# Ouranosinc/xclim

Measured on AMD Instinct MI355X. Metric: grid-cells x timesteps / s (tx90p = percentile_doy + threshold_count + missing mask), higher is better.
Workload: dtype f32; 1 GPU; tx90p (percentile_doy window 5 per 90 + threshold_count > + MissingAny) on 365x1440x720 fp32 per GPU, noleap, freq YS, time-major, resident in HBM

## Files before the change

xclim_amd/csrc/common.h:

```cpp
#pragma once
#include <hip/hip_runtime.h>
#include <stdint.h>
#include <stdio.h>
#include <string.h>

#include "../../include/xclim_hip.h"

struct xh_ctx {
  int device;
  hipStream_t stream;
  hipEvent_t ev0, ev1;
  hipStream_t stream2;
  hipEvent_t ev_ready[2], ev_done[2];
  hipStream_t copy_in, copy_out;
  hipEvent_t ev_lane;
  void* scratch;
  size_t scratch_bytes;
  char* scratch_host;
  size_t scratch_head;
  void* retired[16];
  char* retired_host[16];
  int nretired;
  void* big;
  size_t big_bytes;
// ... 12 lines not shown
    if (_e != hipSuccess) {                                                                 \
      xh_set_error("%s failed: %s (%s:%d)", #expr, hipGetErrorString(_e), __FILE__, __LINE__); \
      (void)hipGetLastError();   \
      return XH_ERR_HIP;                                                                    \
    }                                                                                       \
  } while (0)

#define XH_REQUIRE(cond, code, ...) \
  do {                              \
    if (!(cond)) {                  \
      xh_set_error(__VA_ARGS__);    \
      return (code);                \
    }                               \
  } while (0)

#define XH_LAUNCH_CHECK()                                                                      \
  do {                                                                                         \
    hipError_t _e = hipGetLastError();                                                         \
    if (_e != hipSuccess) {                                                                    \
      xh_set_error("kernel launch failed: %s (%s:%d)", hipGetErrorString(_e), __FILE__, __LINE__); \
      return XH_ERR_HIP;                                                                       \
    }                                                                                          \
  } while (0)

int xh_nanmax_fix(xh_ctx* ctx, const float* x, int64_t T, int64_t C, int64_t st, int64_t sc, int nq, float* out);
int xh_correction_fix(xh_ctx* ctx, const float* ref, const float* hist, int64_t T, int64_t C, int64_t st, int64_t sc, int nq, int kind,
                      float* af, float* hist_q);
int xh_scratch_upload(xh_ctx* ctx, size_t* cursor, const void* host, size_t bytes, void** dptr);
int xh_big_scratch(xh_ctx* ctx, size_t bytes, void** dptr);
int xh_const_rows(xh_ctx* ctx, int64_t elems, const float** nan_row, const float** ninf_row, const float** pinf_row);
int xh_launch_tcount_doy(xh_ctx* ctx, const float* x, int64_t T, int64_t C, int64_t st, int op, const double* table,
                         int64_t tstride, const int32_t* tidx, const int64_t* d_seg, const int64_t* h_seg, int P, int ndoy,
                         int32_t* count_out, int32_t* valid_out);
int xh_qdm_columns(xh_ctx* ctx, const float* xcols, int64_t T, int64_t ncols, int64_t col_stride, const float* af, int64_t af_qs,
                   const double* d_q, int nq, int kind, int interp, int extrap, float* out, int64_t out_cs);
int xh_qdm_sorted_ws(int64_t T, int64_t ncols, size_t* bytes);
int xh_qdm_sorted(xh_ctx* ctx, const float* xcols, int64_t T, int64_t ncols, int64_t col_stride, const float* af, int64_t af_qs,
                  const double* d_q, int nq, int kind, int interp, int extrap, float* out, int64_t out_cs, void* ws);
int xh_qdm_regsort(xh_ctx* ctx, const float* sim, int64_t T, int64_t C, int64_t st, const float* af, int64_t af_qs,
                   const double* d_q, int nq, int kind, int extrap, float* scen, int64_t ost);
int xh_cut_classify(xh_ctx* ctx, const float* sim, int64_t T, int64_t C, int64_t st, const float* gcut, const float* gfac, int ntest,
                    int kind, float* scen, int64_t ost);
int xh_qdm_hist(xh_ctx* ctx, const float* sim, int64_t T, int64_t C, int64_t st, const float* af, int64_t af_qs, const double* d_q,
                int nq, int kind, int extrap, float* scen, int64_t ost);
int xh_tcount_plan(int64_t T, int64_t C, int64_t st, int op, int P, int ndoy, int64_t longest, size_t* lds, int* narrow);
int64_t xh_tcount_meta_slots(int64_t T);
int64_t xh_tcount_slot_of_row(int64_t t);
int xh_tcount_run(xh_ctx* ctx, const float* x, int64_t T, int64_t C, int64_t st, int op, const double* table, int64_t tstride,
                  const uint32_t* meta, int P, int ndoy, int narrow, size_t lds, int32_t* count_out, int32_t* valid_out);
int xh_select_columns(xh_ctx* ctx, const float* xcols, int64_t T, int64_t ncols, int64_t col_stride, const double* d_q,
                      int nq, float* out, int64_t out_cstride, int64_t out_qstride);
int xh_select_columns_lean(xh_ctx* ctx, const float* xcols, int64_t T, int64_t ncols, int64_t col_stride,
                           const double* d_q, int nq, float* out, int64_t out_cstride, int64_t out_qstride);
int xh_select_columns_radix(xh_ctx* ctx, const float* xcols, int64_t T, int64_t ncols, int64_t col_stride, const double* d_q,
                            int nq, float* out, int64_t out_cstride, int64_t out_qstride);
int xh_select_regsort(xh_ctx* ctx, const float* x, int64_t T, int64_t C, int64_t st, const double* d_q, int nq, float* out,
                      int64_t out_cstride, int64_t out_qstride);
int xh_select_hist(xh_ctx* ctx, const float* x, int64_t T, int64_t C, int64_t st, const double* d_q, int nq, float* out,
                   int64_t out_cstride, int64_t out_qstride);
int xh_select_time_major(xh_ctx* ctx, const float* x, int64_t T, int64_t C, int64_t st, const double* d_q, int nq,
                         float* out, int64_t out_cstride, int64_t out_qstride);

__host__ __device__ static inline int64_t cdiv64(int64_t a, int64_t b) { return (a + b - 1) / b; }

#define XH_BLOCK 256

// ... 212 lines not shown
```

xclim_amd/csrc/quantile.hip:

```cpp
#include <stdlib.h>

#include <type_traits>

#include "pdoy.h"

template <typename Getter>
__device__ __forceinline__ double xh_hf_quantile(int L, int n, double q, double alpha, double beta, Getter get) {
  if (L == 1) return (double)get(0);
  if (n < 2) {
    return n == 1 ? (double)get(0) : xh_nan64();
  }
  double nn = (double)n;
  double vi = nn * q + (alpha + q * (1.0 - alpha - beta)) - 1.0;
  if (vi >= nn - 1.0) return (double)get(n - 1);
  if (vi < 0.0) {
    const float v0 = get(0);
    return (v0 - v0 != 0.0f) ? (double)get(n - 1) : (double)v0;
  }
  double prev = floor(vi);
  int ip = (int)prev;
  double gamma = vi - prev;
  float left = get(ip), right = get(ip + 1);
  float diff = right - left;
  double r = (double)left + (double)diff * gamma;
// ... 67 lines not shown
        return xh_key2f(r);
      };
      for (int j = 0; j < nper; ++j) {
        double r = xh_hf_quantile(N, nvalid[v], qs[j], alpha, beta, get);
        out[((int64_t)j * ndoy + d) * C + c + v] = r;
      }
    }
  }
}

__device__ __forceinline__ void ce(uint32_t& a, uint32_t& b) {
  uint32_t lo = a < b ? a : b, hi = a < b ? b : a;
  a = lo;
  b = hi;
}

template <int W>
__device__ __forceinline__ void sort_small(uint32_t (&k)[W]) {
  if (W == 1) return;
  if (W == 2) { ce(k[0], k[1 % W]); return; }
  if (W == 3) { ce(k[0], k[1 % W]); ce(k[1 % W], k[2 % W]); ce(k[0], k[1 % W]); return; }
  if (W == 5) {
    ce(k[0], k[1 % W]); ce(k[3 % W], k[4 % W]); ce(k[2 % W], k[4 % W]); ce(k[2 % W], k[3 % W]); ce(k[0], k[3 % W]);
    ce(k[0], k[2 % W]); ce(k[1 % W], k[4 % W]); ce(k[1 % W], k[3 % W]); ce(k[1 % W], k[2 % W]);
    return;
  }
#pragma unroll
  for (int r = 0; r < W; ++r) {
#pragma unroll
    for (int i = (r & 1); i + 1 < W; i += 2) ce(k[i], k[i + 1]);
  }
}

template <int W, int VEC, bool COUNT = false>
__global__ void __launch_bounds__(XH_BLOCK)
k_pdoy_slide(const float* __restrict__ x, int64_t T, int64_t C, int64_t st, int64_t t_first, int ndoy, int chunk,
             const QTab* __restrict__ qtab, int nper, double* __restrict__ out, int fast, int op = 0,
             const int32_t* __restrict__ doy_period = nullptr, int32_t* __restrict__ cnt_out = nullptr,
             int32_t* __restrict__ valid_out = nullptr) {
  __shared__ QTab s_tab[8 * (W + 1)];
  for (int i = threadIdx.x; i < nper * (W + 1); i += XH_BLOCK) s_tab[i] = qtab[i];
  __syncthreads();
  constexpr int NP = VEC == 4 ? 2 : 1;
  constexpr int GW = VEC == 4 ? 2 : 1;
  const int lane = threadIdx.x & 63;
  const int64_t wbase = ((int64_t)blockIdx.x * XH_BLOCK + (threadIdx.x & ~63)) * VEC;
  if (wbase >= C) return;
  int64_t cg[NP];
  bool okg[NP];
#pragma unroll
  for (int g = 0; g < NP; ++g) {
    cg[g] = wbase + (VEC == 4 ? 2 * lane + 128 * g : lane);
    okg[g] = cg[g] < C;
  }
  auto cell = [&](int v) -> int64_t { return cg[v / GW] + v % GW; };
  constexpr int half = W / 2;
  int d0 = blockIdx.y * chunk, d1 = d0 + chunk;
  if (d1 > ndoy) d1 = ndoy;
  uint32_t win[VEC][W];
  int n[VEC];
#pragma unroll
  for (int v = 0; v < VEC; ++v) {
    n[v] = 0;
#pragma unroll
    for (int k = 0; k < W; ++k) win[v][k] = 0xFFFFFFFFu;
  }
  auto fetch = [&](int64_t t) -> VecF<VEC> {
    const int64_t tc = t < 0 ? 0 : (t >= T ? T - 1 : t);
    const float* row = x + tc * st;
    VecF<VEC> r;
#pragma unroll
    for (int g = 0; g < NP; ++g) {
      const VecF<GW> h = xh_load<GW>(row + (okg[g] ? cg[g] : C - GW));
#pragma unroll
// ... 499 lines not shown
    hipLaunchKernelGGL((k_pdoy_reg<16, 1>), grid, dim3(XH_BLOCK), 0, ctx->stream, x, T, C, st, d_tbase, nyears, ndoy,
                       window, d_q, nper, alpha, beta, out);
  } else if (N <= 32) {
    dim3 grid((unsigned)cdiv64(C, XH_BLOCK), gy);
    hipLaunchKernelGGL((k_pdoy_reg<32, 1>), grid, dim3(XH_BLOCK), 0, ctx->stream, x, T, C, st, d_tbase, nyears, ndoy,
                       window, d_q, nper, alpha, beta, out);
  } else {
    return launch_pdoy_lds(ctx, x, T, C, st, d_tbase, nyears, ndoy, window, d_q, nper, alpha, beta, out, nullptr, T, nullptr,
                           0);
  }
  XH_LAUNCH_CHECK();
  return XH_OK;
}

static int slide_fast_mode(const QTab* tab, int nper, int W) {
  bool allmax = W > 1, allmin = W > 1;
  for (int j = 0; j < nper; ++j) {
    const QTab& e = tab[j * (W + 1) + W];
    allmax = allmax && e.lo == e.hi && e.lo == W - 1;
    allmin = allmin && e.lo == e.hi && e.lo == 0;
  }
  return allmax ? 1 : (allmin ? 2 : 0);
}

static int pdoy_impl(xh_ctx* ctx, const float* x, int64_t T, int64_t C, int64_t st, const int32_t* tbase, int nyears,
                     int ndoy, int window, const double* qh, int nper, double alpha, double beta, const int32_t* vmap,
                     int64_t Tv, double* out) {
  size_t cur = 0;
  void *d_tb = nullptr, *d_q = nullptr, *d_vmap = nullptr;
  const int N = nyears * window;
  bool contiguous = !vmap && nyears == 1 && nper <= 8 && (window == 3 || window == 5 || window == 7) && tbase[0] >= 0;
  for (int d = 1; contiguous && d < ndoy; ++d) contiguous = tbase[d] == tbase[0] + d;
  if (contiguous) {
    QTab tab[8 * 8];
    build_qtab(window, qh, nper, alpha, beta, tab);
    void* d_tab = nullptr;
    int rc = xh_scratch_upload(ctx, &cur, tab, sizeof(QTab) * (size_t)nper * (window + 1), &d_tab);
    if (rc) return rc;
    int chunk = 32;
    if (const char* e = xh_diag_env("XH_PDOY_SLIDE_CHUNK")) chunk = atoi(e) > 0 ? atoi(e) : chunk;
    const int vec = slide_vec(x, C, st, out);
    dim3 grid((unsigned)cdiv64(cdiv64(C, vec), XH_BLOCK), (unsigned)((ndoy + chunk - 1) / chunk));
#define XH_SLIDE(W, V)                                                                                              \
  hipLaunchKernelGGL((k_pdoy_slide<W, V>), grid, dim3(XH_BLOCK), 0, ctx->stream, x, T, C, st, (int64_t)tbase[0], ndoy, \
                     chunk, (const QTab*)d_tab, nper, out, slide_fast_mode(tab, nper, window))
    if (vec == 4) {
      if (window == 3) XH_SLIDE(3, 4); else if (window == 5) XH_SLIDE(5, 4); else XH_SLIDE(7, 4);
    } else {
      if (window == 3) XH_SLIDE(3, 1); else if (window == 5) XH_SLIDE(5, 1); else XH_SLIDE(7, 1);
    }
#undef XH_SLIDE
    XH_LAUNCH_CHECK();
    return XH_OK;
  }
  int rc = xh_scratch_upload(ctx, &cur, tbase, sizeof(int32_t) * (size_t)nyears * ndoy, &d_tb);
  if (rc) return rc;
  rc = xh_scratch_upload(ctx, &cur, qh, sizeof(double) * nper, &d_q);
  if (rc) return rc;
  if (vmap) {
    rc = xh_scratch_upload(ctx, &cur, vmap, sizeof(int32_t) * (size_t)Tv, &d_vmap);
    if (rc) return rc;
  }
  if (!vmap && N <= 32)
    return launch_pdoy(ctx, x, T, C, st, (const int32_t*)d_tb, nyears, ndoy, window, (const double*)d_q, nper, alpha, beta,
                       out);
  const bool mergeable = N > 32 && nyears <= 64 && (window == 3 || window == 5 || window == 7) && nper <= 16;
  if (!mergeable)
    return launch_pdoy_lds(ctx, x, T, C, st, (const int32_t*)d_tb, nyears, ndoy, window, (const double*)d_q, nper, alpha,
                           beta, out, (const int32_t*)d_vmap, Tv, nullptr, 0);
  uint8_t* regular = (uint8_t*)malloc((size_t)ndoy);
  int32_t* irregular = (int32_t*)malloc(sizeof(int32_t) * (size_t)ndoy);
  QTab* tab = (QTab*)malloc(sizeof(QTab) * (size_t)nper * (N + 1));
  if (!regular || !irregular || !tab) {
    free(regular); free(irregular); free(tab);
    xh_set_error("xh_percentile_doy: out of host memory");
    return XH_ERR_ARG;
  }
  const int nirr = pdoy_regular_flags(tbase, nyears, ndoy, window, T, vmap, Tv, regular, irregular);
// ... 76 lines not shown
                                         hipFuncAttributeMaxDynamicSharedMemorySize, (int)lds));                           \
      hipLaunchKernelGGL((k_pdoy_merge<W, NY, false>), grid, dim3(64), lds, ctx->stream, x, T, C, st, (const int32_t*)d_tb, \
                         nyears, ndoy, chunk, (const QTab*)d_tab, (const int32_t*)d_jrest, nrest, out,                      \
                         (const int32_t*)d_vmap, Tv, (const uint8_t*)d_reg, (const int32_t*)nullptr, 0, KT, KB, abl);       \
    }                                                                                                                      \
    if (nirr) {                                                                                                            \
      if (lds_a > 64 * 1024)                                                                                               \
        XH_CHECK_HIP(hipFuncSetAttribute((const void*)k_pdoy_merge<W, NY, true>,                                           \
                                         hipFuncAttributeMaxDynamicSharedMemorySize, (int)lds_a));                         \
      hipLaunchKernelGGL((k_pdoy_merge<W, NY, true>), grid_irr, dim3(64), lds_a, ctx->stream, x, T, C, st,                  \
                         (const int32_t*)d_tb, nyears, ndoy, chunk, (const QTab*)d_tab, (const int32_t*)d_jall, nper, out,  \
                         (const int32_t*)d_vmap, Tv, (const uint8_t*)d_reg, (const int32_t*)d_irr, nirr, KTa, KBa, abl);    \
    }                                                                                                                      \
  } while (0)
  if (NYP == 32) {
    if (window == 3) XH_MERGE(3, 32); else if (window == 5) XH_MERGE(5, 32); else XH_MERGE(7, 32);
  } else {
    if (window == 3) XH_MERGE(3, 64); else if (window == 5) XH_MERGE(5, 64); else XH_MERGE(7, 64);
  }
#undef XH_MERGE
  XH_LAUNCH_CHECK();
  return XH_OK;
}

static int pdoy_count_impl(xh_ctx* ctx, const float* x, int64_t T, int64_t C, int64_t st, const int32_t* tbase, int ndoy,
                           int window, double per, double alpha, double beta, int op, const int32_t* doy_period, int P,
                           int32_t* count_out, int32_t* valid_out) {
  bool contiguous = (window == 3 || window == 5 || window == 7) && tbase[0] >= 0;
  for (int d = 1; contiguous && d < ndoy; ++d) contiguous = tbase[d] == tbase[0] + d;
  if (!contiguous) return XH_ERR_NOTIMPL;
  for (int d = 0; d < ndoy; ++d)
    XH_REQUIRE(doy_period[d] >= 0 && doy_period[d] < P, XH_ERR_ARG, "xh_percentile_doy_count: doy_period[%d] outside [0, P)", d);
  size_t cur = 0;
  QTab tab[8];
  const double q = per / 100.0;
  build_qtab(window, &q, 1, alpha, beta, tab);
  void *d_tab = nullptr, *d_dp = nullptr;
  int rc = xh_scratch_upload(ctx, &cur, tab, sizeof(QTab) * (size_t)(window + 1), &d_tab);
  if (!rc) rc = xh_scratch_upload(ctx, &cur, doy_period, sizeof(int32_t) * (size_t)ndoy, &d_dp);
  if (rc) return rc;
  XH_CHECK_HIP(hipMemsetAsync(count_out, 0, sizeof(int32_t) * (size_t)P * (size_t)C, ctx->stream));
  if (valid_out) XH_CHECK_HIP(hipMemsetAsync(valid_out, 0, sizeof(int32_t) * (size_t)P * (size_t)C, ctx->stream));
  int chunk = 61;
  if (const char* e = xh_diag_env("XH_PDOY_SLIDE_COUNT_CHUNK")) chunk = atoi(e) > 0 ? atoi(e) : chunk;
  const int vec = slide_vec(x, C, st, nullptr);
  dim3 grid((unsigned)cdiv64(cdiv64(C, vec), XH_BLOCK), (unsigned)((ndoy + chunk - 1) / chunk));
#define XH_SLIDEC(W, V)                                                                                                   \
  hipLaunchKernelGGL((k_pdoy_slide<W, V, true>), grid, dim3(XH_BLOCK), 0, ctx->stream, x, T, C, st, (int64_t)tbase[0], ndoy, \
                     chunk, (const QTab*)d_tab, 1, (double*)nullptr, slide_fast_mode(tab, 1, window), op,          \
                     (const int32_t*)d_dp, count_out, valid_out)
  if (vec == 4) {
    if (window == 3) XH_SLIDEC(3, 4); else if (window == 5) XH_SLIDEC(5, 4); else XH_SLIDEC(7, 4);
  } else {
    if (window == 3) XH_SLIDEC(3, 1); else if (window == 5) XH_SLIDEC(5, 1); else XH_SLIDEC(7, 1);
  }
#undef XH_SLIDEC
  XH_LAUNCH_CHECK();
  return XH_OK;
}

static int pdoy_count_multi(xh_ctx* ctx, const float* x, int64_t T, int64_t C, int64_t st, const int32_t* tbase, int nyears,
                            int ndoy, int window, double per, double alpha, double beta, int op, const int32_t* doy_period,
                            int P, int32_t* count_out, int32_t* valid_out) {
  const int N = nyears * window;
  if (!(N > 32 && nyears <= 64 && (window == 3 || window == 5 || window == 7))) return XH_ERR_NOTIMPL;
  if (op != XH_OP_GT && op != XH_OP_GE && op != XH_OP_LT && op != XH_OP_LE) return XH_ERR_NOTIMPL;
  for (int64_t i = 0; i < (int64_t)nyears * ndoy; ++i) {
    XH_REQUIRE(tbase[i] >= -1 && tbase[i] < T, XH_ERR_ARG, "xh_percentile_doy_count: tbase entry out of range");
    XH_REQUIRE(tbase[i] < 0 ? doy_period[i] < 0 : (doy_period[i] >= 0 && doy_period[i] < P), XH_ERR_ARG,
               "xh_percentile_doy_count: doy_period[%lld] must be in [0, P) for present days and < 0 for absent ones",
               (long long)i);
  }
  uint8_t* regular = (uint8_t*)malloc((size_t)ndoy);
  int32_t* irregular = (int32_t*)malloc(sizeof(int32_t) * (size_t)ndoy);
  QTab* tab = (QTab*)malloc(sizeof(QTab) * (size_t)(N + 1));
  if (!regular || !irregular || !tab) {
    free(regular); free(irregular); free(tab);
    xh_set_error("xh_percentile_doy_count: out of host memory");
    return XH_ERR_ARG;
  }
  const int nirr = pdoy_regular_flags(tbase, nyears, ndoy, window, T, nullptr, T, regular, irregular);
  const double q = per / 100.0;
// ... 188 lines not shown
```

xclim_amd/csrc/reduce.hip:

```cpp
#include "common.h"
#include "window.h"

template <int VEC, int KIND>
__global__ void __launch_bounds__(XH_BLOCK)
k_threshold_count(const float* __restrict__ x, int64_t C, int64_t st, int op, float thr32, double thr64,
                  const void* __restrict__ table, int64_t tstride, const int32_t* __restrict__ tidx,
                  const int64_t* __restrict__ seg_off, int P, int32_t* __restrict__ count_out,
                  int32_t* __restrict__ valid_out, int period_fast) {
  const unsigned tile = period_fast ? blockIdx.y : blockIdx.x;
  const int pstart = period_fast ? blockIdx.x : blockIdx.y, pstep = period_fast ? gridDim.x : gridDim.y;
  int64_t c = ((int64_t)tile * XH_BLOCK + threadIdx.x) * VEC;
  if (c >= C) return;
  for (int p = pstart; p < P; p += pstep) {
    int64_t t0 = seg_off[p], t1 = seg_off[p + 1];
    int cnt[VEC], val[VEC];
#pragma unroll
    for (int i = 0; i < VEC; ++i) cnt[i] = 0, val[i] = 0;
    xh_march_rows<VEC, 8>(x + c, st, t0, t1, [&](int64_t t, const VecF<VEC>& xv) {
      if (KIND == XH_THR_SCALAR_F32) {
#pragma unroll
        for (int i = 0; i < VEC; ++i) cnt[i] += xh_cmp_f32(xv.v[i], op, thr32) ? 1 : 0;
      } else if (KIND == XH_THR_SCALAR_F64) {
#pragma unroll
        for (int i = 0; i < VEC; ++i) cnt[i] += xh_cmp_f64((double)xv.v[i], op, thr64) ? 1 : 0;
// ... 170 lines not shown
        else if (RED == XH_RED_VAR) r = (poisoned || n[i] == 0) ? xh_nan32() : (float)(s2[i] / (double)n[i]);
        else r = (poisoned || n[i] == 0) ? xh_nan32() : (float)sqrt(s2[i] / (double)n[i]);
        if (len == 0 && RED != XH_RED_SUM) r = xh_nan32();
        reinterpret_cast<float*>(out_v)[o + i] = r;
      }
    }
    if (valid_out) {
#pragma unroll
      for (int i = 0; i < VEC; ++i) valid_out[o + i] = n[i];
    }
  }
}

template <int VEC>
static int launch_resample_reduce(xh_ctx* ctx, int reducer, dim3 grid, const float* x, int64_t C, int64_t st, int skipna,
                                  const int64_t* seg, int P, void* out, int32_t* valid_out) {
#define XH_RR(R)                                                                                                   \
  case R:                                                                                                          \
    hipLaunchKernelGGL((k_resample_reduce<VEC, R>), grid, dim3(XH_BLOCK), 0, ctx->stream, x, C, st, skipna, seg, P, out, \
                       valid_out);                                                                                 \
    break;
  switch (reducer) {
    XH_RR(XH_RED_SUM) XH_RR(XH_RED_MEAN) XH_RR(XH_RED_MIN) XH_RR(XH_RED_MAX) XH_RR(XH_RED_STD) XH_RR(XH_RED_VAR)
    XH_RR(XH_RED_COUNT) XH_RR(XH_RED_ARGMIN) XH_RR(XH_RED_ARGMAX)
    default:
      xh_set_error("xh_resample_reduce: reducer %d not recognized", reducer);
      return XH_ERR_OP;
  }
#undef XH_RR
  XH_LAUNCH_CHECK();
  return XH_OK;
}

__global__ void __launch_bounds__(XH_BLOCK)
k_apply_missing_mask(const void* __restrict__ value, int kind, const int32_t* __restrict__ valid,
                     const int32_t* __restrict__ expected, int P, int64_t C, double* __restrict__ out) {
  int64_t i = (int64_t)blockIdx.x * XH_BLOCK + threadIdx.x;
  int64_t n = (int64_t)P * C;
  if (i >= n) return;
  int p = (int)(i / C);
  double v = kind == 0 ? (double)reinterpret_cast<const int32_t*>(value)[i]
             : kind == 1 ? (double)reinterpret_cast<const float*>(value)[i]
                         : reinterpret_cast<const double*>(value)[i];
  out[i] = (valid[i] != expected[p]) ? xh_nan64() : v;
}

template <int RED>
__global__ void __launch_bounds__(XH_BLOCK)
k_rolling_reduce(const float* __restrict__ x, int64_t T, int64_t C, int64_t st, int window, int left, int right,
                 float* __restrict__ out, int64_t out_st) {
  int64_t c = (int64_t)blockIdx.x * XH_BLOCK + threadIdx.x;
  if (c >= C) return;
  int64_t chunk = cdiv64(T, (int64_t)gridDim.y);
  int64_t ta = (int64_t)blockIdx.y * chunk, tb = ta + chunk;
  if (tb > T) tb = T;
  for (int64_t t = ta; t < tb; ++t) {
    int64_t a = t - left, b = t + right;
    float r;
    if (RED == XH_RED_COUNT) {
      int n = 0;
      for (int64_t k = (a < 0 ? 0 : a); k <= b && k < T; ++k) {
        float v = x[k * st + c];
        n += (v == v) ? 1 : 0;
      }
      r = (float)n;
    } else if (a < 0 || b >= T) {
      r = xh_nan32();
    } else {
      double s = 0.0;
      float e = x[a * st + c];
      bool nan = false;
      for (int64_t k = a; k <= b; ++k) {
        float v = x[k * st + c];
        nan |= (v != v);
        if (RED == XH_RED_MIN) e = v < e ? v : e;
        else if (RED == XH_RED_MAX) e = v > e ? v : e;
        else s += (double)v;
      }
      if (RED == XH_RED_SUM) r = (float)s;
      else if (RED == XH_RED_MEAN) r = (float)(s / (double)window);
      else if (RED == XH_RED_MIN || RED == XH_RED_MAX) r = e;
      else {
        double m = s / (double)window, s2 = 0.0;
        for (int64_t k = a; k <= b; ++k) {
          double d = (double)x[k * st + c] - m;
          s2 += d * d;
        }
        r = (RED == XH_RED_VAR) ? (float)(s2 / (double)window) : (float)sqrt(s2 / (double)window);
      }
      if (nan) r = xh_nan32();
    }
    out[t * out_st + c] = r;
  }
}

static int check_tc(const char* fn, xh_ctx* ctx, const void* x, int64_t T, int64_t C, int64_t st, int64_t sc) {
  XH_REQUIRE(ctx && x, XH_ERR_ARG, "%s: NULL argument", fn);
  XH_REQUIRE(T >= 0 && C >= 0, XH_ERR_ARG, "%s: negative shape", fn);
  XH_REQUIRE(sc == 1 && st >= C, XH_ERR_LAYOUT,
             "%s: streaming kernels need a time-major view (sc == 1, st >= C); got st=%lld sc=%lld — transpose first",
             fn, (long long)st, (long long)sc);
  return XH_OK;
}

static int upload_segments(xh_ctx* ctx, size_t* cur, const int64_t* seg_off, int P, int64_t T, const char* fn,
                           const int64_t** d_seg) {
  XH_REQUIRE(seg_off && P >= 1, XH_ERR_ARG, "%s: seg_off NULL or P < 1", fn);
  for (int p = 0; p < P; ++p)
    XH_REQUIRE(seg_off[p] <= seg_off[p + 1] && seg_off[p] >= 0 && seg_off[p + 1] <= T, XH_ERR_ARG,
               "%s: seg_off must be non-decreasing within [0, T]", fn);
  void* d = nullptr;
  int rc = xh_scratch_upload(ctx, cur, seg_off, sizeof(int64_t) * (size_t)(P + 1), &d);
  if (rc) return rc;
  *d_seg = (const int64_t*)d;
  return XH_OK;
}

extern "C" {

static int threshold_count_impl(xh_ctx* ctx, const float* x, int64_t T, int64_t C, int64_t st, int64_t sc, int op, int thr_kind,
                                double thr_scalar, const void* thr_table, int64_t thr_stride, const int32_t* tidx,
                                const int64_t* seg_off, int P, int32_t* count_out, int32_t* valid_out, int ndoy) {
  int rc = check_tc("xh_threshold_count", ctx, x, T, C, st, sc);
  if (rc) return rc;
  XH_REQUIRE(op >= XH_OP_GT && op <= XH_OP_NE, XH_ERR_OP, "Operation `%d` not recognized.", op);
  XH_REQUIRE(count_out, XH_ERR_ARG, "xh_threshold_count: count_out is NULL");
  if (thr_kind >= XH_THR_DOY_F64) {
    XH_REQUIRE(thr_table && thr_stride >= C, XH_ERR_ARG, "xh_threshold_count: threshold table missing or stride < C");
    if (thr_kind == XH_THR_DOY_F64 || thr_kind == XH_THR_DOY_F32)
      XH_REQUIRE(tidx, XH_ERR_ARG, "xh_threshold_count: tidx required for per-doy thresholds");
  }
  size_t cur = 0;
  const int64_t* d_seg = nullptr;
  rc = upload_segments(ctx, &cur, seg_off, P, T, "xh_threshold_count", &d_seg);
  if (rc) return rc;
  if (C == 0) return XH_OK;
  if (thr_kind == XH_THR_DOY_F64 && ndoy > 0 && !xh_diag_env("XH_TCOUNT_LEGACY")) {
    rc = xh_launch_tcount_doy(ctx, x, T, C, st, op, static_cast<const double*>(thr_table), thr_stride, tidx, d_seg, seg_off, P,
                              ndoy, count_out, valid_out);
    if (rc != XH_ERR_NOTIMPL) return rc;
  }
  int vec = xh_pick_vec(x, C, st);
  if (thr_kind >= XH_THR_DOY_F64) {
    size_t esz = (thr_kind == XH_THR_DOY_F64 || thr_kind == XH_THR_FULL_F64) ? 8 : 4;
    if ((reinterpret_cast<uintptr_t>(thr_table) & 15) != 0 || (thr_stride * esz) % 16 != 0) vec = 1;
  }
  unsigned tiles = (unsigned)cdiv64(cdiv64(C, vec), XH_BLOCK);
  const bool doy = thr_kind == XH_THR_DOY_F64 || thr_kind == XH_THR_DOY_F32;
  const int period_fast = (doy && P > 1 && tiles <= 65535u) ? 1 : 0;
  dim3 grid = period_fast ? dim3(period_grid(P), tiles) : dim3(tiles, period_grid(P));
  if (vec == 4)
    return launch_threshold_count<4>(ctx, thr_kind, grid, x, C, st, op, thr_scalar, thr_table, thr_stride, tidx, d_seg, P,
                                     count_out, valid_out, period_fast);
  return launch_threshold_count<1>(ctx, thr_kind, grid, x, C, st, op, thr_scalar, thr_table, thr_stride, tidx, d_seg, P,
                                   count_out, valid_out, period_fast);
}

int xh_threshold_count(xh_ctx* ctx, const float* x, int64_t T, int64_t C, int64_t st, int64_t sc, int op, int thr_kind,
                       double thr_scalar, const void* thr_table, int64_t thr_stride, const int32_t* tidx,
                       const int64_t* seg_off, int P, int32_t* count_out, int32_t* valid_out) {
  return threshold_count_impl(ctx, x, T, C, st, sc, op, thr_kind, thr_scalar, thr_table, thr_stride, tidx, seg_off, P, count_out,
                              valid_out, 0);
}

int xh_threshold_count_doy(xh_ctx* ctx, const float* x, int64_t T, int64_t C, int64_t st, int64_t sc, int op,
                           const double* thr_table, int64_t thr_stride, int ndoy, const int32_t* tidx, const int64_t* seg_off,
                           int P, int32_t* count_out, int32_t* valid_out) {
  XH_REQUIRE(ndoy >= 1, XH_ERR_ARG, "xh_threshold_count_doy: the table needs at least one row (ndoy = %d)", ndoy);
  return threshold_count_impl(ctx, x, T, C, st, sc, op, XH_THR_DOY_F64, 0.0, thr_table, thr_stride, tidx, seg_off, P, count_out,
// ... 24 lines not shown
    hipLaunchKernelGGL((k_domain_count<4, true>), grid, dim3(XH_BLOCK), 0, ctx->stream, x, C, st, s1, c1.thr, s2, c2.thr, combine,
                       d_seg, P, count_out, valid_out);
  } else if (vec == 4)
    hipLaunchKernelGGL((k_domain_count<4>), grid, dim3(XH_BLOCK), 0, ctx->stream, x, C, st, op1, (float)thr1, op2,
                       (float)thr2, combine, d_seg, P, count_out, valid_out);
  else
    hipLaunchKernelGGL((k_domain_count<1>), grid, dim3(XH_BLOCK), 0, ctx->stream, x, C, st, op1, (float)thr1, op2,
                       (float)thr2, combine, d_seg, P, count_out, valid_out);
  XH_LAUNCH_CHECK();
  return XH_OK;
}

int xh_resample_reduce(xh_ctx* ctx, const float* x, int64_t T, int64_t C, int64_t st, int64_t sc, int reducer, int skipna,
                       const int64_t* seg_off, int P, void* out, int32_t* valid_out) {
  int rc = check_tc("xh_resample_reduce", ctx, x, T, C, st, sc);
  if (rc) return rc;
  XH_REQUIRE(out, XH_ERR_ARG, "xh_resample_reduce: out is NULL");
  size_t cur = 0;
  const int64_t* d_seg = nullptr;
  rc = upload_segments(ctx, &cur, seg_off, P, T, "xh_resample_reduce", &d_seg);
  if (rc) return rc;
  if (C == 0) return XH_OK;
  int vec = xh_pick_vec(x, C, st);
  dim3 grid((unsigned)cdiv64(cdiv64(C, vec), XH_BLOCK), period_grid(P));
  if (vec == 4) return launch_resample_reduce<4>(ctx, reducer, grid, x, C, st, skipna, d_seg, P, out, valid_out);
  return launch_resample_reduce<1>(ctx, reducer, grid, x, C, st, skipna, d_seg, P, out, valid_out);
}

int xh_apply_missing_mask(xh_ctx* ctx, const void* value, int value_kind, const int32_t* valid, const int32_t* expected,
                          int P, int64_t C, double* out64) {
  XH_REQUIRE(ctx && value && valid && expected && out64, XH_ERR_ARG, "xh_apply_missing_mask: NULL argument");
  XH_REQUIRE(value_kind >= 0 && value_kind <= 2, XH_ERR_ARG, "xh_apply_missing_mask: value_kind must be 0, 1 or 2");
  XH_REQUIRE(P >= 1 && C >= 0, XH_ERR_ARG, "xh_apply_missing_mask: bad shape");
  size_t cur = 0;
  void* d_exp = nullptr;
  int rc = xh_scratch_upload(ctx, &cur, expected, sizeof(int32_t) * (size_t)P, &d_exp);
  if (rc) return rc;
  int64_t n = (int64_t)P * C;
  if (n == 0) return XH_OK;
  hipLaunchKernelGGL(k_apply_missing_mask, dim3((unsigned)cdiv64(n, XH_BLOCK)), dim3(XH_BLOCK), 0, ctx->stream, value,
                     value_kind, valid, (const int32_t*)d_exp, P, C, out64);
  XH_LAUNCH_CHECK();
  return XH_OK;
}

int xh_rolling_reduce(xh_ctx* ctx, const float* x, int64_t T, int64_t C, int64_t st, int64_t sc, int window, int center,
                      int reducer, float* out, int64_t out_st) {
  int rc = check_tc("xh_rolling_reduce", ctx, x, T, C, st, sc);
  if (rc) return rc;
  XH_REQUIRE(out && out_st >= C, XH_ERR_ARG, "xh_rolling_reduce: out NULL or out_st < C");
  XH_REQUIRE(window >= 1, XH_ERR_ARG, "xh_rolling_reduce: window must be >= 1");
  if (T == 0 || C == 0) return XH_OK;
  int left = center ? window / 2 : window - 1;
  int right = window - 1 - left;
  {
    int rr = xh_launch_rolling_ring(ctx, x, T, C, st, window, left, right, reducer, out, out_st);
    if (rr != XH_ERR_NOTIMPL) return rr;
  }
  unsigned ny = (unsigned)(T < 64 ? T : 64);
  dim3 grid((unsigned)cdiv64(C, XH_BLOCK), ny);
#define XH_RO(R)                                                                                                      \
  case R:                                                                                                             \
    hipLaunchKernelGGL((k_rolling_reduce<R>), grid, dim3(XH_BLOCK), 0, ctx->stream, x, T, C, st, window, left, right, out, \
                       out_st);                                                                                       \
    break;
  switch (reducer) {
    XH_RO(XH_RED_SUM) XH_RO(XH_RED_MEAN) XH_RO(XH_RED_MIN) XH_RO(XH_RED_MAX) XH_RO(XH_RED_STD) XH_RO(XH_RED_VAR)
    XH_RO(XH_RED_COUNT)
    default:
      xh_set_error("xh_rolling_reduce: reducer %d not recognized", reducer);
      return XH_ERR_OP;
  }
#undef XH_RO
  XH_LAUNCH_CHECK();
// ... 5 lines not shown
```

xclim_amd/csrc/tcount.hip:

```cpp
#include "f32thr.h"
#include "rowstream.h"

namespace {

constexpr int TC_CW = 64, TC_RL = 16, TC_U = 16, TC_NT = TC_CW * TC_RL, TC_ROWS = TC_RL * TC_U;

__global__ void k_tc_meta(const int32_t* __restrict__ tidx, const int64_t* __restrict__ seg, int P, int64_t T, int64_t nslots,
                          int ndoy, uint32_t* __restrict__ meta) {
  const int64_t i = (int64_t)blockIdx.x * blockDim.x + threadIdx.x;
  if (i >= nslots) return;
  const int64_t kb = i >> 8;
  const int rl = (int)(i >> 4) & 15, u = (int)i & 15;
  const int64_t t = kb * TC_ROWS + u * TC_RL + rl;
  uint32_t dy = (uint32_t)ndoy, per = (uint32_t)P;
  if (t < T) {
    const int d = tidx[t];
    if (d >= 0 && d < ndoy) dy = (uint32_t)d;
    if (t >= seg[0] && t < seg[P]) {
      int lo = 0, hi = P;
      while (hi - lo > 1) {
        const int mid = (lo + hi) >> 1;
        if (seg[mid] <= t) lo = mid; else hi = mid;
      }
      per = (uint32_t)lo;
    }
  }
  meta[i] = dy | (per << 16);
}

template <int OP>
__device__ __forceinline__ bool tc_cmp(float x, float thr) {
  return OP == XH_OP_GT ? x > thr : OP == XH_OP_LT ? x < thr : OP == XH_OP_GE ? x >= thr : x <= thr;
// ... 59 lines not shown
#pragma unroll
        for (int u = 0; u < TC_U; ++u) sum += h[u];
        acc += sum;
      } else {
#pragma unroll
        for (int u = 0; u < TC_U; ++u) {
          const uint32_t pp = m[u] >> 16;
          if (pp != cur) {
            flush(cur, acc);
            acc = 0u;
            cur = pp;
          }
          acc += h[u];
        }
      }
    });
    flush(cur, acc);
    __syncthreads();
    for (int i = tid; i < P * TC_CW; i += TC_NT) {
      const int64_t c2 = tile * TC_CW + (i & (TC_CW - 1));
      const uint32_t w = NARROW ? (cnt[i >> 1] >> ((i & 1) * 16)) & 0xFFFFu : cnt[i];
      if (c2 < C) {
        const int64_t o = (int64_t)(i / TC_CW) * C + c2;
        count_out[o] = (int32_t)(w & (VONE - 1u));
        if (valid_out) valid_out[o] = (int32_t)(w >> VSH);
      }
    }
    __syncthreads();
    for (int i = tid; i < (P + 1) * TC_CW / CPW; i += TC_NT) cnt[i] = 0u;
    __syncthreads();
  }
}

}

int xh_tcount_plan(int64_t T, int64_t C, int64_t st, int op, int P, int ndoy, int64_t longest, size_t* lds, int* narrow) {
  if (op < XH_OP_GT || op > XH_OP_LE) return XH_ERR_NOTIMPL;
  if (ndoy < 1 || ndoy > 0xFFFE || P < 1 || P > 0xFFFE || T > 0x7FFFFFFF) return XH_ERR_NOTIMPL;
  if (longest > 0xFFFF) return XH_ERR_NOTIMPL;
  *narrow = longest <= 0xFF ? 1 : 0;
  *lds = (size_t)(ndoy + 1) * TC_CW * 4 + (size_t)(P + 1) * TC_CW * (*narrow ? 2 : 4);
  if (*lds > 156 * 1024) return XH_ERR_NOTIMPL;
  if (T < 2048 || T < 3 * (int64_t)ndoy || C < TC_CW) return XH_ERR_NOTIMPL;
  if ((int64_t)TC_ROWS * st * 4 >= ((int64_t)1 << 32) || C * 4 + (int64_t)TC_RL * st * 4 >= ((int64_t)1 << 32)) return XH_ERR_NOTIMPL;
  return XH_OK;
}

int64_t xh_tcount_meta_slots(int64_t T) { return (T + TC_ROWS - 1) / TC_ROWS * TC_ROWS; }

int64_t xh_tcount_slot_of_row(int64_t t) {
  const int64_t kb = t / TC_ROWS, r = t % TC_ROWS;
  return (kb * TC_RL + r % TC_RL) * TC_U + r / TC_RL;
}

int xh_tcount_run(xh_ctx* ctx, const float* x, int64_t T, int64_t C, int64_t st, int op, const double* table, int64_t tstride,
                  const uint32_t* meta, int P, int ndoy, int narrow, size_t lds, int32_t* count_out, int32_t* valid_out) {
  const int64_t ntiles = cdiv64(C, TC_CW);
  const unsigned grid = (unsigned)(ntiles < ctx->num_cu ? ntiles : ctx->num_cu);
#define XH_TCD2(OPV, NW)                                                                                                      \
  {                                                                                                                           \
    XH_CHECK_HIP(hipFuncSetAttribute((const void*)k_tc_doy<OPV, NW>, hipFuncAttributeMaxDynamicSharedMemorySize, (int)lds)); \
    hipLaunchKernelGGL((k_tc_doy<OPV, NW>), dim3(grid), dim3(TC_NT), lds, ctx->stream, x, (int)T, C, st, table, tstride, meta,  \
                       ndoy, P, count_out, valid_out);                                                                        \
  }
#define XH_TCD(OPV)                         \
  case OPV:                                 \
    if (narrow) XH_TCD2(OPV, true) else XH_TCD2(OPV, false) \
    break;
  switch (op) {
    XH_TCD(XH_OP_GT)
    XH_TCD(XH_OP_LT)
    XH_TCD(XH_OP_GE)
    XH_TCD(XH_OP_LE)
  }
#undef XH_TCD2
#undef XH_TCD
  XH_LAUNCH_CHECK();
  return XH_OK;
}

int xh_launch_tcount_doy(xh_ctx* ctx, const float* x, int64_t T, int64_t C, int64_t st, int op, const double* table,
                         int64_t tstride, const int32_t* tidx, const int64_t* d_seg, const int64_t* h_seg, int P, int ndoy,
                         int32_t* count_out, int32_t* valid_out) {
  int64_t longest = 0;
  for (int p = 0; p < P; ++p) longest = h_seg[p + 1] - h_seg[p] > longest ? h_seg[p + 1] - h_seg[p] : longest;
  size_t lds = 0;
  int narrow = 0;
  int rc = xh_tcount_plan(T, C, st, op, P, ndoy, longest, &lds, &narrow);
  if (rc) return rc;
  const int64_t nslots = xh_tcount_meta_slots(T);
  void* scratch = nullptr;
  rc = xh_big_scratch(ctx, (size_t)nslots * 4, &scratch);
  if (rc) return rc;
  uint32_t* meta = static_cast<uint32_t*>(scratch);
  hipLaunchKernelGGL(k_tc_meta, dim3((unsigned)cdiv64(nslots, 256)), dim3(256), 0, ctx->stream, tidx, d_seg, P, T, nslots, ndoy, meta);
  return xh_tcount_run(ctx, x, T, C, st, op, table, tstride, meta, P, ndoy, narrow, lds, count_out, valid_out);
}
```

Baseline: 231.0 billion cell-timesteps/s.

## Pass small tables by value and add short-series threshold-count kernel

Quantile tables and missing-mask expected counts now travel as by-value kernel arguments instead of being uploaded to scratch, which removes host-to-device copies before each launch. A new k_tc_year kernel handles short series (T < 2048) with per-year segment offsets passed by value. It double-buffers row loads in reverse time order and accumulates counts in LDS via atomics, skipping the meta-building kernel and segment upload. This adds a second code path and larger kernel argument blocks.

```diff
diff --git a/xclim_amd/csrc/common.h b/xclim_amd/csrc/common.h
--- a/xclim_amd/csrc/common.h
+++ b/xclim_amd/csrc/common.h
@@ -68,6 +68,9 @@
 int xh_launch_tcount_doy(xh_ctx* ctx, const float* x, int64_t T, int64_t C, int64_t st, int op, const double* table,
                          int64_t tstride, const int32_t* tidx, const int64_t* d_seg, const int64_t* h_seg, int P, int ndoy,
                          int32_t* count_out, int32_t* valid_out);
+int xh_launch_tcount_year(xh_ctx* ctx, const float* x, int64_t T, int64_t C, int64_t st, int op, const double* table,
+                          int64_t tstride, const int32_t* tidx, const int64_t* h_seg, int P, int ndoy, int32_t* count_out,
+                          int32_t* valid_out);
 int xh_qdm_columns(xh_ctx* ctx, const float* xcols, int64_t T, int64_t ncols, int64_t col_stride, const float* af, int64_t af_qs,
                    const double* d_q, int nq, int kind, int interp, int extrap, float* out, int64_t out_cs);
 int xh_qdm_sorted_ws(int64_t T, int64_t ncols, size_t* bytes);
diff --git a/xclim_amd/csrc/quantile.hip b/xclim_amd/csrc/quantile.hip
--- a/xclim_amd/csrc/quantile.hip
+++ b/xclim_amd/csrc/quantile.hip
@@ -123,14 +123,18 @@
   }
 }
 
+struct QTabArg {
+  QTab e[8 * 8];
+};
+
 template <int W, int VEC, bool COUNT = false>
 __global__ void __launch_bounds__(XH_BLOCK)
 k_pdoy_slide(const float* __restrict__ x, int64_t T, int64_t C, int64_t st, int64_t t_first, int ndoy, int chunk,
-             const QTab* __restrict__ qtab, int nper, double* __restrict__ out, int fast, int op = 0,
+             const QTabArg qtab, int nper, double* __restrict__ out, int fast, int op = 0,
              const int32_t* __restrict__ doy_period = nullptr, int32_t* __restrict__ cnt_out = nullptr,
              int32_t* __restrict__ valid_out = nullptr) {
   __shared__ QTab s_tab[8 * (W + 1)];
-  for (int i = threadIdx.x; i < nper * (W + 1); i += XH_BLOCK) s_tab[i] = qtab[i];
+  for (int i = threadIdx.x; i < nper * (W + 1); i += XH_BLOCK) s_tab[i] = qtab.e[i];
   __syncthreads();
   constexpr int NP = VEC == 4 ? 2 : 1;
   constexpr int GW = VEC == 4 ? 2 : 1;
@@ -696,18 +700,16 @@
   bool contiguous = !vmap && nyears == 1 && nper <= 8 && (window == 3 || window == 5 || window == 7) && tbase[0] >= 0;
   for (int d = 1; contiguous && d < ndoy; ++d) contiguous = tbase[d] == tbase[0] + d;
   if (contiguous) {
-    QTab tab[8 * 8];
+    QTabArg qa;
+    QTab* tab = qa.e;
     build_qtab(window, qh, nper, alpha, beta, tab);
-    void* d_tab = nullptr;
-    int rc = xh_scratch_upload(ctx, &cur, tab, sizeof(QTab) * (size_t)nper * (window + 1), &d_tab);
-    if (rc) return rc;
     int chunk = 32;
     if (const char* e = xh_diag_env("XH_PDOY_SLIDE_CHUNK")) chunk = atoi(e) > 0 ? atoi(e) : chunk;
     const int vec = slide_vec(x, C, st, out);
     dim3 grid((unsigned)cdiv64(cdiv64(C, vec), XH_BLOCK), (unsigned)((ndoy + chunk - 1) / chunk));
 #define XH_SLIDE(W, V)                                                                                              \
   hipLaunchKernelGGL((k_pdoy_slide<W, V>), grid, dim3(XH_BLOCK), 0, ctx->stream, x, T, C, st, (int64_t)tbase[0], ndoy, \
-                     chunk, (const QTab*)d_tab, nper, out, slide_fast_mode(tab, nper, window))
+                     chunk, qa, nper, out, slide_fast_mode(tab, nper, window))
     if (vec == 4) {
       if (window == 3) XH_SLIDE(3, 4); else if (window == 5) XH_SLIDE(5, 4); else XH_SLIDE(7, 4);
     } else {
@@ -850,12 +852,12 @@
   for (int d = 0; d < ndoy; ++d)
     XH_REQUIRE(doy_period[d] >= 0 && doy_period[d] < P, XH_ERR_ARG, "xh_percentile_doy_count: doy_period[%d] outside [0, P)", d);
   size_t cur = 0;
-  QTab tab[8];
+  QTabArg qa;
+  QTab* tab = qa.e;
   const double q = per / 100.0;
   build_qtab(window, &q, 1, alpha, beta, tab);
-  void *d_tab = nullptr, *d_dp = nullptr;
-  int rc = xh_scratch_upload(ctx, &cur, tab, sizeof(QTab) * (size_t)(window + 1), &d_tab);
-  if (!rc) rc = xh_scratch_upload(ctx, &cur, doy_period, sizeof(int32_t) * (size_t)ndoy, &d_dp);
+  void* d_dp = nullptr;
+  int rc = xh_scratch_upload(ctx, &cur, doy_period, sizeof(int32_t) * (size_t)ndoy, &d_dp);
   if (rc) return rc;
   XH_CHECK_HIP(hipMemsetAsync(count_out, 0, sizeof(int32_t) * (size_t)P * (size_t)C, ctx->stream));
   if (valid_out) XH_CHECK_HIP(hipMemsetAsync(valid_out, 0, sizeof(int32_t) * (size_t)P * (size_t)C, ctx->stream));
@@ -865,7 +867,7 @@
   dim3 grid((unsigned)cdiv64(cdiv64(C, vec), XH_BLOCK), (unsigned)((ndoy + chunk - 1) / chunk));
 #define XH_SLIDEC(W, V)                                                                                                   \
   hipLaunchKernelGGL((k_pdoy_slide<W, V, true>), grid, dim3(XH_BLOCK), 0, ctx->stream, x, T, C, st, (int64_t)tbase[0], ndoy, \
-                     chunk, (const QTab*)d_tab, 1, (double*)nullptr, slide_fast_mode(tab, 1, window), op,          \
+                     chunk, qa, 1, (double*)nullptr, slide_fast_mode(tab, 1, window), op,                          \
                      (const int32_t*)d_dp, count_out, valid_out)
   if (vec == 4) {
     if (window == 3) XH_SLIDEC(3, 4); else if (window == 5) XH_SLIDEC(5, 4); else XH_SLIDEC(7, 4);
diff --git a/xclim_amd/csrc/reduce.hip b/xclim_amd/csrc/reduce.hip
--- a/xclim_amd/csrc/reduce.hip
+++ b/xclim_amd/csrc/reduce.hip
@@ -226,9 +226,14 @@
   return XH_OK;
 }
 
+struct XhExpected {
+  int32_t v[64];
+};
+
+template <bool BYVAL>
 __global__ void __launch_bounds__(XH_BLOCK)
 k_apply_missing_mask(const void* __restrict__ value, int kind, const int32_t* __restrict__ valid,
-                     const int32_t* __restrict__ expected, int P, int64_t C, double* __restrict__ out) {
+                     const int32_t* __restrict__ expected, const XhExpected exv, int P, int64_t C, double* __restrict__ out) {
   int64_t i = (int64_t)blockIdx.x * XH_BLOCK + threadIdx.x;
   int64_t n = (int64_t)P * C;
   if (i >= n) return;
@@ -236,7 +241,7 @@
   double v = kind == 0 ? (double)reinterpret_cast<const int32_t*>(value)[i]
              : kind == 1 ? (double)reinterpret_cast<const float*>(value)[i]
                          : reinterpret_cast<const double*>(value)[i];
-  out[i] = (valid[i] != expected[p]) ? xh_nan64() : v;
+  out[i] = (valid[i] != (BYVAL ? exv.v[p] : expected[p])) ? xh_nan64() : v;
 }
 
 template <int RED>
@@ -297,14 +302,20 @@
   return XH_OK;
 }
 
-static int upload_segments(xh_ctx* ctx, size_t* cur, const int64_t* seg_off, int P, int64_t T, const char* fn,
-                           const int64_t** d_seg) {
+static int check_segments(const int64_t* seg_off, int P, int64_t T, const char* fn) {
   XH_REQUIRE(seg_off && P >= 1, XH_ERR_ARG, "%s: seg_off NULL or P < 1", fn);
   for (int p = 0; p < P; ++p)
     XH_REQUIRE(seg_off[p] <= seg_off[p + 1] && seg_off[p] >= 0 && seg_off[p + 1] <= T, XH_ERR_ARG,
                "%s: seg_off must be non-decreasing within [0, T]", fn);
+  return XH_OK;
+}
+
+static int upload_segments(xh_ctx* ctx, size_t* cur, const int64_t* seg_off, int P, int64_t T, const char* fn,
+                           const int64_t** d_seg) {
+  int rc = check_segments(seg_off, P, T, fn);
+  if (rc) return rc;
   void* d = nullptr;
-  int rc = xh_scratch_upload(ctx, cur, seg_off, sizeof(int64_t) * (size_t)(P + 1), &d);
+  rc = xh_scratch_upload(ctx, cur, seg_off, sizeof(int64_t) * (size_t)(P + 1), &d);
   if (rc) return rc;
   *d_seg = (const int64_t*)d;
   return XH_OK;
@@ -324,11 +335,18 @@
     if (thr_kind == XH_THR_DOY_F64 || thr_kind == XH_THR_DOY_F32)
       XH_REQUIRE(tidx, XH_ERR_ARG, "xh_threshold_count: tidx required for per-doy thresholds");
   }
+  rc = check_segments(seg_off, P, T, "xh_threshold_count");
+  if (rc) return rc;
+  if (C == 0) return XH_OK;
+  if (thr_kind == XH_THR_DOY_F64 && ndoy > 0 && !xh_diag_env("XH_TCOUNT_LEGACY")) {
+    rc = xh_launch_tcount_year(ctx, x, T, C, st, op, static_cast<const double*>(thr_table), thr_stride, tidx, seg_off, P, ndoy,
+                               count_out, valid_out);
+    if (rc != XH_ERR_NOTIMPL) return rc;
+  }
   size_t cur = 0;
   const int64_t* d_seg = nullptr;
   rc = upload_segments(ctx, &cur, seg_off, P, T, "xh_threshold_count", &d_seg);
   if (rc) return rc;
-  if (C == 0) return XH_OK;
   if (thr_kind == XH_THR_DOY_F64 && ndoy > 0 && !xh_diag_env("XH_TCOUNT_LEGACY")) {
     rc = xh_launch_tcount_doy(ctx, x, T, C, st, op, static_cast<const double*>(thr_table), thr_stride, tidx, d_seg, seg_off, P,
                               ndoy, count_out, valid_out);
@@ -419,14 +437,25 @@
   XH_REQUIRE(ctx && value && valid && expected && out64, XH_ERR_ARG, "xh_apply_missing_mask: NULL argument");
   XH_REQUIRE(value_kind >= 0 && value_kind <= 2, XH_ERR_ARG, "xh_apply_missing_mask: value_kind must be 0, 1 or 2");
   XH_REQUIRE(P >= 1 && C >= 0, XH_ERR_ARG, "xh_apply_missing_mask: bad shape");
-  size_t cur = 0;
+  XhExpected exv;
+  const bool byval = P <= 64;
   void* d_exp = nullptr;
-  int rc = xh_scratch_upload(ctx, &cur, expected, sizeof(int32_t) * (size_t)P, &d_exp);
-  if (rc) return rc;
+  if (byval) {
+    memset(&exv, 0, sizeof(exv));
+    memcpy(exv.v, expected, sizeof(int32_t) * (size_t)P);
+  } else {
+    size_t cur = 0;
+    int rc = xh_scratch_upload(ctx, &cur, expected, sizeof(int32_t) * (size_t)P, &d_exp);
+    if (rc) return rc;
+  }
   int64_t n = (int64_t)P * C;
   if (n == 0) return XH_OK;
-  hipLaunchKernelGGL(k_apply_missing_mask, dim3((unsigned)cdiv64(n, XH_BLOCK)), dim3(XH_BLOCK), 0, ctx->stream, value,
-                     value_kind, valid, (const int32_t*)d_exp, P, C, out64);
+  if (byval)
+    hipLaunchKernelGGL(k_apply_missing_mask<true>, dim3((unsigned)cdiv64(n, XH_BLOCK)), dim3(XH_BLOCK), 0, ctx->stream, value,
+                       value_kind, valid, (const int32_t*)nullptr, exv, P, C, out64);
+  else
+    hipLaunchKernelGGL(k_apply_missing_mask<false>, dim3((unsigned)cdiv64(n, XH_BLOCK)), dim3(XH_BLOCK), 0, ctx->stream, value,
+                       value_kind, valid, (const int32_t*)d_exp, exv, P, C, out64);
   XH_LAUNCH_CHECK();
   return XH_OK;
 }
diff --git a/xclim_amd/csrc/tcount.hip b/xclim_amd/csrc/tcount.hip
--- a/xclim_amd/csrc/tcount.hip
+++ b/xclim_amd/csrc/tcount.hip
@@ -1,3 +1,5 @@
+#include <stdlib.h>
+
 #include "f32thr.h"
 #include "rowstream.h"
 
@@ -123,6 +125,146 @@
   }
 }
 
+
+constexpr int TY_RL = 8, TY_NT = 64 * TY_RL, TY_CW = 256, TY_PMAX = 64, TY_U = 2;
+
+struct TySeg {
+  int32_t off[TY_PMAX + 1];
+};
+
+template <int OP>
+__device__ __forceinline__ bool ty_cmp(double a, double b) {
+  return OP == XH_OP_GT ? a > b : OP == XH_OP_LT ? a < b : OP == XH_OP_GE ? a >= b : OP == XH_OP_LE ? a <= b
+       : OP == XH_OP_EQ ? a == b : a != b;
+}
+
+struct TyRow {
+  float2 x[2];
+  double2 t[2];
+};
+
+template <int OP, bool REVERSE>
+__global__ void __launch_bounds__(TY_NT)
+k_tc_year(const float* __restrict__ x, int64_t C, int64_t st, const double* __restrict__ table, int64_t tstride,
+          const int32_t* __restrict__ tidx, int ndoy, const TySeg seg, int P, int32_t* __restrict__ count_out,
+          int32_t* __restrict__ valid_out) {
+  extern __shared__ __attribute__((aligned(16))) unsigned char smem[];
+  uint32_t* cnt = reinterpret_cast<uint32_t*>(smem);
+  const int tid = threadIdx.x, lane = tid & 63;
+  const int rl = __builtin_amdgcn_readfirstlane(tid >> 6);
+  const int64_t tile0 = (int64_t)blockIdx.x * TY_CW;
+  for (int i = tid; i < P * TY_CW; i += TY_NT) cnt[i] = 0u;
+  uint32_t off[2];
+#pragma unroll
+  for (int g = 0; g < 2; ++g) {
+    const int64_t c = tile0 + 2 * lane + 128 * g;
+    off[g] = (uint32_t)(c < C ? c : C - 2);
+  }
+  const int t0 = seg.off[0], t1 = seg.off[P];
+  const int n = t1 - t0;
+  const int nk = n > rl ? (n - rl + TY_RL - 1) / TY_RL : 0;
+  const int nb = (nk + TY_U - 1) / TY_U;
+  __syncthreads();
+  auto row_of = [&](int k) -> int {
+    k = k < nk ? k : nk - 1;
+    return REVERSE ? t1 - 1 - rl - k * TY_RL : t0 + rl + k * TY_RL;
+  };
+  auto doy_of = [&](int b, int (&d)[TY_U]) {
+#pragma unroll
+    for (int u = 0; u < TY_U; ++u) d[u] = tidx[row_of(b * TY_U + u)];
+  };
+  auto load = [&](TyRow (&dst)[TY_U], bool (&bad)[TY_U], int b, const int (&d)[TY_U]) {
+#pragma unroll
+    for (int u = 0; u < TY_U; ++u) {
+      const int t = row_of(b * TY_U + u);
+      bad[u] = (unsigned)d[u] >= (unsigned)ndoy;
+      const int dd = bad[u] ? 0 : d[u];
+      const float* xr = x + (int64_t)t * st;
+      const double* tr = table + (int64_t)dd * tstride;
+#pragma unroll
+      for (int g = 0; g < 2; ++g) {
+        dst[u].x[g] = *reinterpret_cast<const float2*>(xr + off[g]);
+        dst[u].t[g] = *reinterpret_cast<const double2*>(tr + off[g]);
+      }
+    }
+  };
+  uint32_t acc[4] = {0u, 0u, 0u, 0u};
+  int p = REVERSE ? P - 1 : 0;
+  int bound = REVERSE ? seg.off[P - 1] : seg.off[1];
+  auto flush = [&]() {
+    uint32_t* c = cnt + p * TY_CW + 2 * lane;
+#pragma unroll
+    for (int v = 0; v < 4; ++v) {
+      atomicAdd(&c[(v >> 1) * 128 + (v & 1)], acc[v]);
+      acc[v] = 0u;
+    }
+  };
+  auto consume = [&](const TyRow (&r)[TY_U], const bool (&bad)[TY_U], int b) {
+#pragma unroll
+    for (int u = 0; u < TY_U; ++u) {
+      const int k = b * TY_U + u;
+      if (k >= nk) break;
+      const int t = row_of(k);
+      if (REVERSE ? t < bound : t >= bound) {
+        flush();
+        if (REVERSE) {
+          do { --p; } while (t < seg.off[p]);
+          bound = seg.off[p];
+        } else {
+          do { ++p; } while (t >= seg.off[p + 1]);
+          bound = seg.off[p + 1];
+        }
+      }
+#pragma unroll
+      for (int g = 0; g < 2; ++g) {
+        const float xv[2] = {r[u].x[g].x, r[u].x[g].y};
+        const double tv[2] = {r[u].t[g].x, r[u].t[g].y};
+#pragma unroll
+        for (int j = 0; j < 2; ++j) {
+          const bool h = bad[u] ? OP == XH_OP_NE : ty_cmp<OP>((double)xv[j], tv[j]);
+          acc[2 * g + j] += (h ? 1u : 0u) + (xv[j] == xv[j] ? 0x10000u : 0u);
+        }
+      }
+    }
+  };
+  if (nb > 0) {
+    TyRow A[TY_U], B[TY_U];
+    bool badA[TY_U], badB[TY_U];
+    int d[TY_U];
+    doy_of(0, d);
+    load(A, badA, 0, d);
+    doy_of(1, d);
+    int b = 0;
+    while (b + 2 < nb) {
+      load(B, badB, b + 1, d);
+      doy_of(b + 2, d);
+      consume(A, badA, b);
+      load(A, badA, b + 2, d);
+      doy_of(b + 3, d);
+      consume(B, badB, b + 1);
+      b += 2;
+    }
+    if (b + 1 < nb) {
+      load(B, badB, b + 1, d);
+      consume(A, badA, b);
+      consume(B, badB, b + 1);
+    } else {
+      consume(A, badA, b);
+    }
+    flush();
+  }
+  __syncthreads();
+  for (int i = tid; i < P * TY_CW; i += TY_NT) {
+    const int64_t c = tile0 + (i & (TY_CW - 1));
+    if (c < C) {
+      const uint32_t w = cnt[i];
+      const int64_t o = (int64_t)(i / TY_CW) * C + c;
+      count_out[o] = (int32_t)(w & 0xFFFFu);
+      if (valid_out) valid_out[o] = (int32_t)(w >> 16);
+    }
+  }
+}
+
 }
 
 int xh_tcount_plan(int64_t T, int64_t C, int64_t st, int op, int P, int ndoy, int64_t longest, size_t* lds, int* narrow) {
@@ -166,6 +308,41 @@
   }
 #undef XH_TCD2
 #undef XH_TCD
+  XH_LAUNCH_CHECK();
+  return XH_OK;
+}
+
+int xh_launch_tcount_year(xh_ctx* ctx, const float* x, int64_t T, int64_t C, int64_t st, int op, const double* table,
+                          int64_t tstride, const int32_t* tidx, const int64_t* h_seg, int P, int ndoy, int32_t* count_out,
+                          int32_t* valid_out) {
+  if (!(T < 2048 || T < 3 * (int64_t)ndoy)) return XH_ERR_NOTIMPL;
+  if (const char* e = xh_diag_env("XH_TCOUNT_YEAR")) if (!atoi(e)) return XH_ERR_NOTIMPL;
+  if (op < XH_OP_GT || op > XH_OP_NE || P < 1 || P > TY_PMAX || T > 0xFFFF || ndoy < 1 || C < 2 || (C & 1) || (st & 1) ||
+      (tstride & 1) || (reinterpret_cast<uintptr_t>(x) & 7) || (reinterpret_cast<uintptr_t>(table) & 15) ||
+      cdiv64(C, TY_CW) > 0x7FFFFFFF)
+    return XH_ERR_NOTIMPL;
+  TySeg seg;
+  for (int p = 0; p <= P; ++p) seg.off[p] = (int32_t)h_seg[p];
+  const bool fwd = [] { const char* e = xh_diag_env("XH_TCOUNT_YEAR_FWD"); return e && atoi(e); }();
+  const size_t lds = (size_t)P * TY_CW * 4;
+  const dim3 grid((unsigned)cdiv64(C, TY_CW));
+#define XH_TY2(OPV, REV) \
+  hipLaunchKernelGGL((k_tc_year<OPV, REV>), grid, dim3(TY_NT), lds, ctx->stream, x, C, st, table, tstride, tidx, ndoy, seg, P, \
+                     count_out, valid_out)
+#define XH_TY(OPV)                           \
+  case OPV:                                  \
+    if (fwd) XH_TY2(OPV, false); else XH_TY2(OPV, true); \
+    break;
+  switch (op) {
+    XH_TY(XH_OP_GT)
+    XH_TY(XH_OP_LT)
+    XH_TY(XH_OP_GE)
+    XH_TY(XH_OP_LE)
+    XH_TY(XH_OP_EQ)
+    XH_TY(XH_OP_NE)
+  }
+#undef XH_TY2
+#undef XH_TY
   XH_LAUNCH_CHECK();
   return XH_OK;
 }
```

After: 230.3 billion cell-timesteps/s (median of 2 runs). Within noise of the previous version (-0.3%).
